# valeoai/rainbow-iqn-apex

Hardware: NVIDIA H100
Metric: learner grad-steps/sec (batch=512, N=N'=64) (higher is better)
Workload: dtype fp16 fwd / bf16 bwd tensor-core products, fp32 accumulate; fp32 elsewhere

## Files before the change

rainbow_iqn_apex_b200/csrc/conv.cu:

```cuda
#include "common.cuh"
#include "gemm.h"
#include "../../include/riqn_b200.h"

namespace riqn {

template <typename T>
__device__ __forceinline__ float load_px(const T* p);
template <>
__device__ __forceinline__ float load_px<uint8_t>(const uint8_t* p) { return (float)(*p) / 255.0f; }
template <>
__device__ __forceinline__ float load_px<float>(const float* p) { return *p; }

template <typename T>
__global__ void im2col_kernel(riqn_conv_geom g, const T* __restrict__ in, float* __restrict__ col) {
  const int K = g.Cin * g.KH * g.KW;
  const long total = (long)g.B * g.OH * g.OW * K;
  for (long idx = (long)blockIdx.x * blockDim.x + threadIdx.x; idx < total; idx += (long)gridDim.x * blockDim.x) {
    const int k = (int)(idx % K);
    const long m = idx / K;
    const int kw = k % g.KW, kh = (k / g.KW) % g.KH, c = k / (g.KW * g.KH);
    const int ow = (int)(m % g.OW), oh = (int)((m / g.OW) % g.OH), b = (int)(m / ((long)g.OW * g.OH));
    const int ih = oh * g.stride + kh - g.pad, iw = ow * g.stride + kw - g.pad;
    float v = 0.f;
    if (ih >= 0 && ih < g.H && iw >= 0 && iw < g.W) v = load_px<T>(&in[(long)b * g.in_bstride + ((long)c * g.H + ih) * g.W + iw]);
// ... 516 lines not shown
          d_[u][h] = on ? __ldg(dout + src) : 0.f;
        }
#pragma unroll
      for (int u = 0; u < 4; ++u) {
        const int c = c0 + 8 * u;
        if (c < Cout) {
          float acc = 0.f;
#pragma unroll
          for (int h = 0; h < 2; ++h) {
            const float v = o_[u][h] > 0.f ? d_[u][h] : 0.f;
            tile[lane + 32 * h][c] = __bfloat16_as_ushort(__float2bfloat16_rn(v));
            acc += v;
          }
          acc = warp_sum(acc);
          if (lane == 0) bsum[c] += acc;
        }
      }
    }
    __syncthreads();
    const int ppr = Cout >> 3;
    for (int idx = threadIdx.x; idx < 64 * ppr; idx += blockDim.x) {
      const int r = idx / ppr, pc = idx - r * ppr;
      if (m0 + r < Mg) {
        const uint32_t* w = reinterpret_cast<const uint32_t*>(&tile[r][pc * 8]);
        *reinterpret_cast<uint4*>(dYg + (m0 + r) * Cout + pc * 8) = make_uint4(w[0], w[1], w[2], w[3]);
      }
    }
    __syncthreads();
  }
  if (threadIdx.x < Cout) dbias_part[(long)blockIdx.x * Cout + threadIdx.x] = bsum[threadIdx.x];
}

__global__ void unpermute_add_kernel(int Cout, int K, const float* __restrict__ dwp, const int* __restrict__ perm,
                                     float* __restrict__ dw) {
  const int idx = blockIdx.x * blockDim.x + threadIdx.x;
  if (idx >= Cout * K) return;
  const int c = idx / K, kp = idx - c * K;
  dw[(long)c * K + perm[kp]] += dwp[idx];
}

static int strip_params(const riqn_conv_geom* g, int* t, int* G, int* kc) {
  if (g->KH != g->KW || g->stride < 1 || g->KH % g->stride) return 1;
  *t = g->KH / g->stride;
  *G = g->OH + *t - 1;
  const int Kc = g->stride * g->stride * g->Cin;
  if (g->OH != g->OW || Kc % 64 || g->OH != (g->H + 2 * g->pad - g->KH) / g->stride + 1) return 1;
  *kc = Kc / 64;
  return 0;
}

RIQN_API int riqn_s2d_u8(const riqn_conv_geom* g, const unsigned char* in, void* a_px, void* stream) {
  riqn::note_launches(1);
  int t, G, kc;
  const int chw = g->Cin * g->H * g->W;
  if (strip_params(g, &t, &G, &kc) || chw % 16 || g->in_bstride % 16 || (reinterpret_cast<uintptr_t>(in) & 15) ||
      chw > 96 * 1024)
    return (int)cudaErrorInvalidValue;
  static PerDeviceOnce attr_once;
  const int attr_dev = PerDeviceOnce::device();
  if (!attr_once.done[attr_dev]) {
    RIQN_CUDA(cudaFuncSetAttribute(s2d_u8_kernel, cudaFuncAttributeMaxDynamicSharedMemorySize, 96 * 1024));
    attr_once.done[attr_dev] = true;
  }
  s2d_u8_kernel<<<g->B, 256, chw, (cudaStream_t)stream>>>(*g, G, in, (bf16*)a_px);
  return (int)cudaGetLastError();
}

RIQN_API int riqn_conv_fwd_strip(const riqn_conv_geom* g, const void* a_hi, const void* a_lo, const void* w_hi,
                                 const void* w_lo, const float* bias, float* out, void* next_hi, void* next_lo,
                                 int next_stride, int next_grid, const void* w2_hi, const void* w2_lo, const float* bias2,
                                 int share_a, void* stream) {
  riqn::note_launches(1);
  int t, G, kc;
  if (strip_params(g, &t, &G, &kc) || g->Cout > 64 || (next_hi && (next_stride < 1 || next_grid < 1)))
    return (int)cudaErrorInvalidValue;
  TcExtra ex;
  if (w2_hi != nullptr) {
    const long rows = (long)g->B * G * G;
    if ((g->B & 1) || (rows / 2) % 128 || bias2 == nullptr || (w_lo != nullptr) != (w2_lo != nullptr)) return (int)cudaErrorInvalidValue;
    ex.grp_mt = (int)(rows / 2 / 128);
    ex.b2_hi = (const bf16*)w2_hi; ex.b2_lo = (const bf16*)w2_lo; ex.bias2 = bias2;
    if (share_a) { ex.a_wrap = 1; ex.a_rows = rows / 2; }
  }
  ex.strip_t = t; ex.strip_G = G; ex.strip_kc = kc;
  ex.cv_oh = g->OH; ex.cv_ow = g->OW;
  ex.nx_hi = (bf16*)next_hi; ex.nx_lo = (bf16*)next_lo; ex.nx_s = next_stride; ex.nx_G = next_grid;
  return gemm_bf16_tc(g->B * G * G, g->Cout, g->Cin * g->KH * g->KW, (const bf16*)a_hi, (const bf16*)a_lo, (const bf16*)w_hi,
                      (const bf16*)w_lo, out, g->Cout, TC_CONV, bias, nullptr, nullptr, 1, (cudaStream_t)stream, &ex);
}

__global__ void col2im_gather_kernel(riqn_conv_geom g, int G, const float* __restrict__ dcol, float* __restrict__ din) {
  const long i = (long)blockIdx.x * blockDim.x + threadIdx.x;
  const long n = (long)g.B * g.Cin * g.H * g.W;
  if (i >= n) return;
  const int c = (int)(i % g.Cin), iw = (int)((i / g.Cin) % g.W), ih = (int)((i / ((long)g.Cin * g.W)) % g.H);
  const long b = i / ((long)g.Cin * g.W * g.H);
  const int K = g.Cin * g.KH * g.KW;
  float acc = 0.f;
  for (int kh = 0; kh < g.KH; ++kh) {
    const int oy = ih - kh;
    if (oy < 0 || oy % g.stride) continue;
    const int oh = oy / g.stride;
    if (oh >= g.OH) continue;
    for (int kw = 0; kw < g.KW; ++kw) {
      const int ox = iw - kw;
      if (ox < 0 || ox % g.stride) continue;
      const int ow = ox / g.stride;
      if (ow >= g.OW) continue;
      acc += dcol[((b * G + oh) * G + ow) * K + (c * g.KH + kh) * g.KW + kw];
    }
  }
  din[((b * g.Cin + c) * g.H + ih) * g.W + iw] = acc;
}

RIQN_API int riqn_conv_bwd_strip(const riqn_conv_geom* g, const float* dout, const float* out, const void* a_hi,
                                 const void* w_hi, const int* perm, void* dYg, float* dwp_scratch, float* dw, float* dbias,
                                 float* din, float wgrad_scale, void* stream) {
  riqn::note_launches(din ? 6 : 4);
  cudaStream_t s = (cudaStream_t)stream;
  int t, G, kc;
  if (strip_params(g, &t, &G, &kc) || g->Cout > 64 || g->Cout % 8 || (din && g->pad != 0)) return (int)cudaErrorInvalidValue;
  const long Mg = (long)g->B * G * G;
  const int K = g->Cin * g->KH * g->KW;
  const long tiles = (Mg + 63) / 64;
  const int dy_grid = (int)(tiles < 4L * riqn_sms() ? tiles : 4L * riqn_sms());
  StreamScratch dbias_part;
  RIQN_CUDA(dbias_part.alloc((size_t)dy_grid * g->Cout, s));
  conv_dy_grid_kernel<<<dy_grid, 256, 0, s>>>(g->B, g->Cout, g->OH, g->OW, G, dout, out, (bf16*)dYg, dbias_part.p);
  RIQN_LAUNCH_CHECK();
  if (int rc_ = sum_slots_add(dy_grid, g->Cout, dbias_part.p, dbias, s)) return rc_;
  RIQN_CUDA(cudaMemsetAsync(dwp_scratch, 0, sizeof(float) * g->Cout * K, s));
  TcExtra ex;
  ex.mn_major = 3;
  ex.wg_t = t; ex.wg_G = G; ex.wg_kc = kc;
  ex.alpha = wgrad_scale;
  const int n_tiles = (K + 127) / 128;
  const int split = tc_pick_split(n_tiles, (Mg + 63) / 64);
  int rc = gemm_bf16_tc(g->Cout, K, (int)Mg, (const bf16*)dYg, nullptr, (const bf16*)a_hi, nullptr, dwp_scratch, K, TC_ATOMIC,
                        nullptr, nullptr, nullptr, split, s, &ex);
  if (rc) return rc;
  unpermute_add_kernel<<<(g->Cout * K + 255) / 256, 256, 0, s>>>(g->Cout, K, dwp_scratch, perm, dw);
  RIQN_LAUNCH_CHECK();
  if (din) {
    StreamScratch dcol_buf;
    RIQN_CUDA(dcol_buf.alloc((size_t)Mg * K, s));
    float* dcol = dcol_buf.p;
    TcExtra ci;
    ci.mn_major = 2;
    rc = gemm_bf16_tc((int)Mg, K, g->Cout, (const bf16*)dYg, nullptr, (const bf16*)w_hi, nullptr, dcol, K, TC_STORE, nullptr,
                      nullptr, nullptr, 1, s, &ci);
    if (rc) return rc;
    const long n_in = (long)g->B * g->Cin * g->H * g->W;
    col2im_gather_kernel<<<riqn_cdiv(n_in, 256), 256, 0, s>>>(*g, G, dcol, din);
    RIQN_LAUNCH_CHECK();
  }
  return 0;
}

RIQN_API int riqn_conv_bwd_tc(const riqn_conv_geom* g, const float* dout, const float* out, const void* colT_hi,
                              const void* wT_hi, void* dY_hi, void* dYT_hi, float* dcol, float* dw, float* dbias, float* din,
                              float wgrad_scale, void* stream) {
  riqn::note_launches(din ? 4 : 2);
  cudaStream_t s = (cudaStream_t)stream;
  const long M = (long)g->B * g->OH * g->OW;
  const int K = g->Cin * g->KH * g->KW;
  const int ohw = g->OH * g->OW;
  if (M % 8 || g->Cout % 8) return (int)cudaErrorInvalidValue;
  const long tiles = (M + 63) / 64;
  const int slots = g->Cout <= 64 ? (int)(tiles < 4L * riqn_sms() ? tiles : 4L * riqn_sms()) : (int)((M + 256 * 8 - 1) / (256 * 8));
  StreamScratch dbias_part;
  RIQN_CUDA(dbias_part.alloc((size_t)slots * g->Cout, s));
  if (g->Cout <= 64) {
    conv_dy_tile_kernel<<<slots, 256, 0, s>>>(g->B, g->Cout, ohw, dout, out, din ? (bf16*)dY_hi : nullptr, (bf16*)dYT_hi,
                                              dbias_part.p);
  } else {
    dim3 grid((unsigned)slots, g->Cout);
    conv_dy_bf16_kernel<<<grid, 256, 0, s>>>(g->B, g->Cout, ohw, dout, out, din ? (bf16*)dY_hi : nullptr, (bf16*)dYT_hi,
                                             dbias_part.p);
  }
  RIQN_LAUNCH_CHECK();
  if (int rc_ = sum_slots_add(slots, g->Cout, dbias_part.p, dbias, s)) return rc_;
  const int n_tiles = (K + 127) / 128;
  int split = (riqn_sms() + n_tiles - 1) / n_tiles;
  TcExtra ex;
  ex.alpha = wgrad_scale;
  int rc = gemm_bf16_tc(g->Cout, K, (int)M, (const bf16*)dYT_hi, nullptr, (const bf16*)colT_hi, nullptr, dw, K, TC_ATOMIC,
                        nullptr, nullptr, nullptr, split, s, &ex);
// ... 22 lines not shown
```

rainbow_iqn_apex_b200/csrc/gemm.h:

```cpp
#pragma once
#include <cuda_bf16.h>
#include <cuda_runtime.h>

#include "common.cuh"

namespace riqn {

enum Epi {
  EPI_STORE = 0,
  EPI_BIAS_RELU = 1,
  EPI_BIAS_RELU_NCHW = 2,
  EPI_EMBED = 3,
  EPI_ATOMIC = 4,
  EPI_NOISY_WGRAD = 5,
  EPI_BIAS = 6,
};

struct EpiArgs {
  const float* bias = nullptr;
  const float* feat = nullptr;
  int batch = 1;
  int ohw = 1;
  float* out2 = nullptr;
  const float* eps = nullptr;
  float alpha = 1.0f;
};

int gemm_f32(int M, int N, int K, const float* A, long sAm, long sAk, const float* B, long sBn, long sBk,
             float* C, long ldc, int epi, const EpiArgs& e, int split_k, cudaStream_t stream);

enum TcEpi { TC_STORE = 0, TC_BIAS_RELU = 1, TC_ATOMIC = 2, TC_NOISY_WGRAD = 3, TC_BIAS_RELU_NCHW = 4, TC_EMBED = 5,
             TC_COL2IM = 6, TC_CONV = 7 };

struct TcExtra {
  int ohw = 1;
  float alpha = 1.0f;
  const float* feat = nullptr;
  int batch = 1;
  __nv_bfloat16 *o_hi = nullptr, *o_lo = nullptr, *o_hiT = nullptr, *o_loT = nullptr;
  int ci_h = 0, ci_w = 0, ci_cin = 0, ci_kh = 0, ci_kw = 0, ci_stride = 0, ci_ow = 0, ci_G = 0, ci_oh = 0;
  int strip_t = 0, strip_G = 0, strip_kc = 0, cv_oh = 0, cv_ow = 0, nx_s = 0, nx_G = 0;
  __nv_bfloat16 *nx_hi = nullptr, *nx_lo = nullptr;
  int mn_major = 0, wg_t = 0, wg_G = 0, wg_kc = 0;
  int fmt = 0;
  int grp_mt = 0, a_wrap = 0;
  long a_rows = 0;
  const __nv_bfloat16 *b2_hi = nullptr, *b2_lo = nullptr;
  const float* bias2 = nullptr;
};

int gemm_bf16_tc(int M, int N, int K, const __nv_bfloat16* A_hi, const __nv_bfloat16* A_lo, const __nv_bfloat16* B_hi,
                 const __nv_bfloat16* B_lo, float* C, long ldc, int epi, const float* bias, float* out2, const float* eps,
                 int split_k, cudaStream_t s, const TcExtra* ex);
inline int tc_max_split(long tiles) {
  if (tiles < 1) tiles = 1;
  const long s = riqn_sms() / tiles;
  return s < 1 ? 1 : (int)s;
}
inline int tc_pick_split(int tiles, long kb) {
  const int s = tc_max_split(tiles);
  return kb < s ? (int)(kb < 1 ? 1 : kb) : s;
}

int split_bf16(long rows, int cols, const float* src, __nv_bfloat16* hi, __nv_bfloat16* lo, __nv_bfloat16* hiT,
               __nv_bfloat16* loT, cudaStream_t s, int fp16 = 0);
// ... 3 lines not shown
```

rainbow_iqn_apex_b200/csrc/gemm_tc.cu:

```cuda
#include <cuda.h>
#include <cudaTypedefs.h>
#include <algorithm>
#include <map>
#include <mutex>
#include <tuple>

#include "common.cuh"
#include "gemm.h"
#include "../../include/riqn_b200.h"

namespace riqn {

using bf16 = __nv_bfloat16;

constexpr int TBM = 128, TBK = 64, MMA_K = 16;
constexpr int kConsumerWGs = 2;
constexpr int kEpiWarps = 4 * kConsumerWGs;
constexpr int kTcThreads = 128 * (1 + kConsumerWGs);
constexpr uint32_t kSlabStride = 72, kSlabBytes = 64 * kSlabStride * 4;
constexpr uint32_t kSmemLimit = 232448;

template <int NSPLIT, int BN, int EPI>
struct TcCfg {
  static constexpr int kAOps = NSPLIT == 3 ? 2 : 1, kBOps = NSPLIT == 1 ? 1 : 2;
// ... 308 lines not shown
  uint64_t* bars = reinterpret_cast<uint64_t*>(smem + Cfg::kStages * Cfg::kStageBytes + Cfg::kEpiBytes);
  uint64_t* full = bars;
  uint64_t* empty = bars + Cfg::kStages;
  const uint32_t epi_base = (uint32_t)__cvta_generic_to_shared(smem + Cfg::kStages * Cfg::kStageBytes);
  const uint32_t epi_fb = epi_base + Cfg::kEpiBytes + 256;

  const int warp = threadIdx.x >> 5, lane = threadIdx.x & 31;
  const int total_units = p.m_tiles * p.n_tiles * p.k_splits;

  if (threadIdx.x == 0) {
    asm volatile("prefetch.tensormap [%0];" ::"l"(reinterpret_cast<uint64_t>(&mapA_hi)) : "memory");
    asm volatile("prefetch.tensormap [%0];" ::"l"(reinterpret_cast<uint64_t>(&mapB_hi)) : "memory");
    if (NSPLIT == 3) asm volatile("prefetch.tensormap [%0];" ::"l"(reinterpret_cast<uint64_t>(&mapA_lo)) : "memory");
    if (NSPLIT >= 2) asm volatile("prefetch.tensormap [%0];" ::"l"(reinterpret_cast<uint64_t>(&mapB_lo)) : "memory");
    for (int i = 0; i < Cfg::kStages; ++i) { mbar_init(&full[i], 1); mbar_init(&empty[i], kEpiWarps); }
    asm volatile("fence.mbarrier_init.release.cluster;" ::: "memory");
  }
  __syncthreads();

  if (warp < 4) {
    if constexpr (BN == 256) asm volatile("setmaxnreg.dec.sync.aligned.u32 40;" ::: "memory");
    if (warp == 0 && lane == 0) {
      int stage = 0;
      uint32_t phase = 0;
      for (int u = blockIdx.x; u < total_units; u += gridDim.x) {
        const int tiles = p.m_tiles * p.n_tiles;
        const int ks = u / tiles, t = u - ks * tiles;
        const int nt = t % p.n_tiles, mt = t / p.n_tiles;
        const int kb0 = ks * p.kb_per_split, kb1 = min(p.kb_total, kb0 + p.kb_per_split);
        for (int kb = kb0; kb < kb1; ++kb) {
          mbar_wait(&empty[stage], phase ^ 1);
          uint8_t* s = smem + stage * Cfg::kStageBytes;
          mbar_expect_tx(&full[stage], Cfg::kStageBytes);
          if (NSPLIT == 1 && p.mn_major) {
            const int kk = kb * TBK;
            if (p.mn_major & 1) {
#pragma unroll
              for (int i = 0; i < TBM / 64; ++i) tma_load_2d(s + i * 8192, &mapA_hi, mt * TBM + 64 * i, kk, &full[stage]);
            } else {
              tma_load_2d(s, &mapA_hi, kk, mt * TBM, &full[stage]);
            }
            if (p.mn_major & 2) {
#pragma unroll
              for (int i = 0; i < (TBN >= 64 ? TBN / 64 : 1); ++i) {
                int b_in = nt * TBN + 64 * i, b_row = kk;
                if (p.wg_t) {
                  const int slab = b_in >> 6, sft = slab / p.wg_kc, dy = sft / p.wg_t;
                  b_in = (slab - sft * p.wg_kc) << 6;
                  b_row += dy * p.wg_G + (sft - dy * p.wg_t);
                }
                tma_load_2d(s + Cfg::kOps * Cfg::kABytes + i * 8192, &mapB_hi, b_in, b_row, &full[stage]);
              }
            } else {
              tma_load_2d(s + Cfg::kOps * Cfg::kABytes, &mapB_hi, kk, nt * TBN, &full[stage]);
            }
            if (++stage == Cfg::kStages) { stage = 0; phase ^= 1; }
            continue;
          }
          int a_col = kb * TBK, a_row = mt * TBM;
          const CUtensorMap *mb_hi = &mapB_hi, *mb_lo = &mapB_lo;
          if (EPI == TC_CONV && p.grp_mt && mt >= p.grp_mt) {
            mb_hi = &p.mapO[0];
            mb_lo = &p.mapO[1];
            if (p.a_wrap) a_row = (mt - p.grp_mt) * TBM;
          }
          if (EPI == TC_CONV) {
// ... 12 lines not shown
    }
    return;
  }

  if constexpr (BN == 256) asm volatile("setmaxnreg.inc.sync.aligned.u32 232;" ::: "memory");
  const int g = (warp >> 2) - 1;
  const int wq = warp & 3;
  const int band = wq & 1, colhalf = wq >> 1;
  const int quarter = 2 * g + band;
  const int ew = warp - 4;
  const uint32_t slab = epi_base + g * kSlabBytes;
  const uint32_t st = slab + wq * (32 * kStRow * 4);
  const bool f16 = (p.fmt & 3) != 0;
  float conv_bias[32];
  if (EPI == TC_CONV) {
#pragma unroll
    for (int j = 0; j < 32; ++j) conv_bias[j] = (32 * colhalf + j < p.N && 32 * colhalf < TBN) ? p.bias[32 * colhalf + j] : 0.f;
  }
  bool conv_grp1 = false;
  int stage = 0;
  uint32_t phase = 0;
  for (int u = blockIdx.x; u < total_units; u += gridDim.x) {
    const int tiles = p.m_tiles * p.n_tiles;
    const int ks = u / tiles, t = u - ks * tiles;
    const int nt = t % p.n_tiles, mt = t / p.n_tiles;
    const int kb0 = ks * p.kb_per_split, kb1 = min(p.kb_total, kb0 + p.kb_per_split);
    if (EPI == TC_CONV && p.grp_mt && (mt >= p.grp_mt) != conv_grp1) {
      conv_grp1 = mt >= p.grp_mt;
      const float* bsrc = conv_grp1 ? p.bias2 : p.bias;
#pragma unroll
      for (int j = 0; j < 32; ++j) conv_bias[j] = (32 * colhalf + j < p.N && 32 * colhalf < TBN) ? bsrc[32 * colhalf + j] : 0.f;
    }
    float acc[TBN / 2];
    int prev = -1;
    for (int kb = kb0; kb < kb1; ++kb) {
      mbar_wait(&full[stage], phase);
      const uint32_t s0 = smem_u32(smem + stage * Cfg::kStageBytes);
      const uint32_t sa = s0 + g * 8192;
      const uint32_t sb = s0 + Cfg::kOps * Cfg::kABytes;
      wgmma_fence();
      if constexpr (BN == 256) {
        mma_kblock<TBN>(acc, sa, sb, kb == kb0, (MODE & 4) != 0, MODE & 3);
      } else if (NSPLIT == 1 && p.mn_major) {
#pragma unroll
        for (int k = 0; k < TBK / MMA_K; ++k) {
          const uint32_t koff_mn = k * (MMA_K / 8) * 1024;
          const uint32_t koff_k = k * MMA_K * 2;
          const uint64_t da = (p.mn_major & 1) ? gmma_desc_mn128(sa + koff_mn) : gmma_desc_k128(sa + koff_k);
          const uint64_t db = (p.mn_major & 2) ? gmma_desc_mn128(sb + koff_mn) : gmma_desc_k128(sb + koff_k);
          wgmma_tile<TBN>(acc, da, db, (kb > kb0 || k > 0) ? 1u : 0u, f16, p.mn_major);
        }
      } else {
#pragma unroll
        for (int k = 0; k < TBK / MMA_K; ++k) {
          const uint32_t koff = k * MMA_K * 2;
          const uint64_t a_hi = gmma_desc_k128(sa + koff), b_hi = gmma_desc_k128(sb + koff);
          wgmma_tile<TBN>(acc, a_hi, b_hi, (kb > kb0 || k > 0) ? 1u : 0u, f16, 0);
          if (NSPLIT >= 2) wgmma_tile<TBN>(acc, a_hi, gmma_desc_k128(sb + Cfg::kBBytes + koff), 1u, false, 0);
          if (NSPLIT == 3) wgmma_tile<TBN>(acc, gmma_desc_k128(sa + Cfg::kABytes + koff), b_hi, 1u, false, 0);
        }
      }
      wgmma_commit();
      wgmma_wait<1>();
      if (prev >= 0) {
        __syncwarp();
        if (lane == 0) mbar_arrive(&empty[prev]);
      }
      prev = stage;
      if (++stage == Cfg::kStages) { stage = 0; phase ^= 1; }
    }
    wgmma_wait<0>();
    __syncwarp();
    if (lane == 0) mbar_arrive(&empty[prev]);

#pragma unroll
    for (int h = 0; h < (TBN + 63) / 64; ++h) {
      if (BN == 256 && nt * TBN + 64 * h >= p.N) break;
      if (EPI == TC_EMBED && lane == 0) tma_store_wait_read();
      wg_bar(1 + g);
      {
        const uint32_t r0 = slab + ((16 * wq + (lane >> 2)) * kSlabStride + 2 * (lane & 3)) * 4;
#pragma unroll
        for (int j = 0; j < 8; ++j) {
          const int jj = 8 * h + j;
          if (jj * 8 < TBN) {
            asm volatile("st.shared.v2.f32 [%0], {%1, %2};" ::"r"(r0 + j * 32), "f"(acc[4 * jj]), "f"(acc[4 * jj + 1]) : "memory");
            asm volatile("st.shared.v2.f32 [%0], {%1, %2};" ::"r"(r0 + 8 * kSlabStride * 4 + j * 32), "f"(acc[4 * jj + 2]),
                         "f"(acc[4 * jj + 3]) : "memory");
          }
        }
      }
      wg_bar(1 + g);
      const int c = 64 * h + 32 * colhalf;
      uint32_t v[32];
      if (c < TBN) {
        const uint32_t rr = slab + ((32 * band + lane) * kSlabStride + 32 * colhalf) * 4;
#pragma unroll
        for (int j = 0; j < 8; ++j) {
          const uint4 x = lds128(rr + 16 * j);
          v[4 * j] = x.x; v[4 * j + 1] = x.y; v[4 * j + 2] = x.z; v[4 * j + 3] = x.w;
        }
      }
      wg_bar(1 + g);
      if (c >= TBN) continue;
      const int m = mt * TBM + quarter * 32 + lane;
      const int n0 = nt * TBN + c;
// ... 15 lines not shown
            for (int j = 0; j < 32; j += 4) {
              float4 o = make_float4(__uint_as_float(v[j]), __uint_as_float(v[j + 1]), __uint_as_float(v[j + 2]),
                                     __uint_as_float(v[j + 3]));
              if (EPI == TC_BIAS_RELU) {
                const float4 b = *reinterpret_cast<const float4*>(p.bias + n0 + j);
                o.x = fmaxf(o.x + b.x, 0.f); o.y = fmaxf(o.y + b.y, 0.f);
                o.z = fmaxf(o.z + b.z, 0.f); o.w = fmaxf(o.w + b.w, 0.f);
              }
              *reinterpret_cast<float4*>(crow + j) = o;
              if (EPI == TC_BIAS_RELU && p.o_hiT) {
                p.o_hiT[(long)(n0 + j) * p.M + m] = __float2bfloat16_rn(o.x);
                p.o_hiT[(long)(n0 + j + 1) * p.M + m] = __float2bfloat16_rn(o.y);
                p.o_hiT[(long)(n0 + j + 2) * p.M + m] = __float2bfloat16_rn(o.z);
                p.o_hiT[(long)(n0 + j + 3) * p.M + m] = __float2bfloat16_rn(o.w);
              }
            }
          } else {
#pragma unroll
            for (int j = 0; j < 32; ++j) {
              if (n0 + j < p.N) {
                float o = __uint_as_float(v[j]);
                if (EPI == TC_BIAS_RELU) o = fmaxf(o + p.bias[n0 + j], 0.f);
                crow[j] = o;
                if (EPI == TC_BIAS_RELU && p.o_hiT) p.o_hiT[(long)(n0 + j) * p.M + m] = __float2bfloat16_rn(o);
              }
            }
          }
        } else if (EPI == TC_BIAS_RELU_NCHW) {
          const int b = m / p.ohw, pp = m - b * p.ohw;
          float* cb = p.C + ((long)b * p.N + n0) * p.ohw + pp;
#pragma unroll
          for (int j = 0; j < 32; ++j)
            if (n0 + j < p.N) cb[(long)j * p.ohw] = fmaxf(__uint_as_float(v[j]) + p.bias[n0 + j], 0.f);
        } else if (EPI == TC_EMBED || EPI == TC_COL2IM || EPI == TC_CONV) {
        } else if (!(p.vec_acc && n0 + 32 <= p.N)) {
          float* crow = p.C + (long)m * p.ldc + n0;
#pragma unroll
          for (int j = 0; j < 32; ++j) {
            if (n0 + j < p.N) {
              const float o = __uint_as_float(v[j]) * (EPI == TC_ATOMIC ? p.alpha : 1.f);
              crow[j] += o;
              if (EPI == TC_NOISY_WGRAD) p.out2[(long)m * p.ldc + n0 + j] += o * p.eps[(long)m * p.ldc + n0 + j];
            }
          }
        }
      }
      if (EPI == TC_CONV && n0 < p.N) {
        const int gg = p.strip_G * p.strip_G;
        const int mm = m < p.M ? m : 0;
        const int b = mm / gg, rem = mm - b * gg;
        const int gy = rem / p.strip_G, gx = rem - gy * p.strip_G;
        const bool valid = m < p.M && gy < p.cv_oh && gx < p.cv_ow;
        float x[32];
#pragma unroll
        for (int j = 0; j < 32; ++j) x[j] = n0 + j < p.N ? fmaxf(__uint_as_float(v[j]) + conv_bias[j], 0.f) : 0.f;
        if (p.C != nullptr && valid) {
          const int plane = p.cv_oh * p.cv_ow;
          float* cb = p.C + ((long)b * p.N + n0) * plane + gy * p.cv_ow + gx;
#pragma unroll
          for (int j = 0; j < 32; ++j)
            if (n0 + j < p.N) cb[(long)j * plane] = x[j];
        }
        if (p.nx_hi != nullptr && n0 + 32 <= p.N) {
          long o = -1;
          if (valid) {
            const int sn = p.nx_s, by = gy / sn, bx = gx / sn;
            const long r = ((long)b * p.nx_G + by) * p.nx_G + bx;
// ... 12 lines not shown
          uint4 pc[8];
          long orow[8];
#pragma unroll
          for (int i = 0; i < 8; ++i) {
            pc[i] = staged_piece(st, 4 * i + sub, piece);
            orow[i] = __shfl_sync(0xffffffffu, o, 4 * i + sub);
          }
#pragma unroll
          for (int i = 0; i < 8; ++i)
            if (orow[i] >= 0 && dstb != nullptr) *reinterpret_cast<uint4*>(dstb + orow[i] + (piece & 3) * 8) = pc[i];
        }
      }
      if (EPI == TC_COL2IM && n0 < p.N) {
        const int khw = p.ci_kh * p.ci_kw;
        const int kcol = n0 + lane;
        int coff = -1;
        if (kcol < p.N) {
          const int c = kcol / khw, r = kcol - c * khw;
          const int kh = r / p.ci_kw, kw = r - kh * p.ci_kw;
          coff = (c * p.ci_h + kh) * p.ci_w + kw;
        }
        bool row_ok = m < p.M;
        const int mm = row_ok ? m : 0;
        const int b = mm / p.ohw, pp = mm - b * p.ohw;
        const int rw = p.ci_G ? p.ci_G : p.ci_ow;
        const int oh = pp / rw, ow = pp - oh * rw;
        if (p.ci_G) row_ok = row_ok && oh < p.ci_oh && ow < p.ci_ow;
        float* base = p.C + ((long)b * p.ci_cin * p.ci_h + oh * p.ci_stride) * p.ci_w + ow * p.ci_stride;
#pragma unroll
        for (int j = 0; j < 32; ++j) {
          const int off = __shfl_sync(0xffffffffu, coff, j);
          if (row_ok && off >= 0)
            asm volatile("red.global.add.f32 [%0], %1;" ::"l"(base + off), "f"(__uint_as_float(v[j])) : "memory");
        }
      }
      if ((EPI == TC_STORE || EPI == TC_EMBED || (EPI == TC_BIAS_RELU && (p.M & 1) == 0) ||
           ((EPI == TC_ATOMIC || EPI == TC_NOISY_WGRAD) && p.vec_acc)) && n0 + 32 <= p.N) {
        const int m_base = mt * TBM + quarter * 32;
        const int rows_valid = min(32, p.M - m_base);
        if (rows_valid > 0) {
          if (EPI == TC_STORE) {
            if (p.o_hi != nullptr) {
              uint32_t hw2[32];
#pragma unroll
              for (int j = 0; j < 16; ++j) {
                const __nv_bfloat162 h2 = __floats2bfloat162_rn(__uint_as_float(v[2 * j]), __uint_as_float(v[2 * j + 1]));
                hw2[j] = *reinterpret_cast<const uint32_t*>(&h2);
                hw2[16 + j] = 0u;
              }
              warp_store_rows_bf16(st, hw2, lane, p.o_hi + (long)m_base * p.N + n0, nullptr, p.N, rows_valid);
            } else {
              warp_store_rows_f32(st, v, lane, p.C + ks * p.part_stride + (long)m_base * p.ldc + n0, p.ldc, rows_valid);
            }
          } else if (EPI == TC_ATOMIC) {
            warp_accum_rows_f32<false>(st, v, lane, p.C + (long)m_base * p.ldc + n0, nullptr, nullptr, p.ldc, rows_valid,
                                       p.alpha);
          } else if (EPI == TC_NOISY_WGRAD) {
            const long o0 = (long)m_base * p.ldc + n0;
            warp_accum_rows_f32<true>(st, v, lane, p.C + o0, p.out2 + o0, p.eps + o0, p.ldc, rows_valid, 1.f);
          } else if (EPI == TC_BIAS_RELU) {
            const float* br = p.bias + n0;
            uint32_t hw[16];
#pragma unroll
            for (int j = 0; j < 32; j += 4) {
              const float4 bb = __ldg(reinterpret_cast<const float4*>(br + j));
              const float x0 = fmaxf(__uint_as_float(v[j]) + bb.x, 0.f), x1 = fmaxf(__uint_as_float(v[j + 1]) + bb.y, 0.f);
// ... 121 lines not shown
    attr_once.sms[attr_dev] = sms;
  }
  const int units = p.m_tiles * p.n_tiles * p.k_splits;
  const int grid = units < sms ? units : sms;
  gemm_tc_kernel<NSPLIT, EPI, BN, MODE><<<grid, kTcThreads, Cfg::kSmemBytes, s>>>(a_hi, a_lo, b_hi, b_lo, p);
  return (int)cudaGetLastError();
}

__global__ void split_k_reduce_kernel(int M, int N, int splits, long stride, long ldp, const float* __restrict__ part,
                                      float* __restrict__ C, long ldc, float alpha, float* __restrict__ out2,
                                      const float* __restrict__ eps) {
  const long i = (long)blockIdx.x * blockDim.x + threadIdx.x;
  if (i >= (long)M * N) return;
  const long m = i / N, n = i - m * N;
  float acc = 0.f;
  for (int k = 0; k < splits; ++k) acc += part[k * stride + m * ldp + n];
  C[m * ldc + n] += alpha * acc;
  if (out2 != nullptr) out2[m * ldc + n] += acc * eps[m * ldc + n];
}

int gemm_bf16_tc(int M, int N, int K, const bf16* A_hi, const bf16* A_lo, const bf16* B_hi, const bf16* B_lo, float* C,
                 long ldc, int epi, const float* bias, float* out2, const float* eps, int split_k, cudaStream_t s,
                 const TcExtra* ex) {
  if (M <= 0 || N <= 0 || K <= 0) return 0;
  if ((K % 8) && !(ex != nullptr && ex->mn_major == 3)) return (int)cudaErrorInvalidValue;
  const bool split3 = A_lo != nullptr && B_lo != nullptr;
  const bool split2 = A_lo == nullptr && B_lo != nullptr;
  const bool narrow_ok = epi == TC_BIAS_RELU_NCHW || epi == TC_CONV || ((epi == TC_ATOMIC || epi == TC_STORE) && !split3 && !split2);
  const bool strip = epi == TC_CONV;
  if (strip && (ex == nullptr || ex->strip_t < 1 || ex->strip_kc < 1 || ex->strip_G < 1 || N > 64 ||
                K != ex->strip_t * ex->strip_t * ex->strip_kc * TBK || (ex->nx_hi && (N % 32))))
    return (int)cudaErrorInvalidValue;
  const long a_k = strip ? (long)ex->strip_kc * TBK : K;
  const bool mn = ex != nullptr && ex->mn_major != 0;
  if (mn) {
    if (split3 || split2 || ((ex->mn_major & 1) && (M % 8)) || ((ex->mn_major & 2) && (N % 8)) ||
        (((ex->mn_major & 3) != 3) && (K % 8)))
      return (int)cudaErrorInvalidValue;
  }
  const long kb_all = (K + TBK - 1) / TBK;
  bool wide = false;
  if (!split3 && !split2 && N > 128 && kb_all >= 16 && (mn ? (ex->mn_major != 1 && ex->wg_t == 0) : !strip) &&
      (epi == TC_STORE || epi == TC_NOISY_WGRAD ||
       (epi == TC_BIAS_RELU && !mn && (ex == nullptr || ex->o_hiT == nullptr)))) {
    const long sms = riqn_sms();
    const long t128 = (long)((M + TBM - 1) / TBM) * ((N + 127) / 128), t256 = (long)((M + TBM - 1) / TBM) * ((N + 255) / 256);
    const bool unsplit = std::min(std::max(split_k, 1), std::min<int>(tc_max_split(t128), (int)kb_all)) == 1;
    wide = (epi != TC_NOISY_WGRAD || unsplit) && (t256 >= sms || 2 * ((t256 + sms - 1) / sms) <= (t128 + sms - 1) / sms);
  }
  const int bn = wide ? 256
                      : (ex != nullptr && ex->mn_major) ? ((narrow_ok && N <= 64) ? 64 : 128)
                                                        : (narrow_ok && N <= 32) ? 32 : (narrow_ok && N <= 64) ? 64 : 128;
  CUtensorMap ma_hi, ma_lo, mb_hi, mb_lo;
  int rc;
  if (mn) {
    const long b_cols = ex->wg_t ? (long)ex->wg_kc * TBK : N;
    rc = (ex->mn_major & 1) ? make_map(&ma_hi, A_hi, K, M, 64) : make_map(&ma_hi, A_hi, M, K, TBM);
    if (rc) return rc;
    rc = (ex->mn_major & 2) ? make_map(&mb_hi, B_hi, K, b_cols, 64) : make_map(&mb_hi, B_hi, N, K, bn);
    if (rc) return rc;
  } else {
    rc = make_map(&ma_hi, A_hi, (ex && ex->a_rows) ? ex->a_rows : M, a_k, TBM);
    if (rc) return rc;
    rc = make_map(&mb_hi, B_hi, N, K, bn);
    if (rc) return rc;
  }
  ma_lo = ma_hi;
  mb_lo = mb_hi;
  if (split3) {
    rc = make_map(&ma_lo, A_lo, (ex && ex->a_rows) ? ex->a_rows : M, a_k, TBM);
    if (rc) return rc;
  }
  if (split3 || split2) {
    rc = make_map(&mb_lo, B_lo, N, K, bn);
    if (rc) return rc;
  }
  TcArgs p;
  p.M = M; p.N = N; p.K = K;
  p.m_tiles = (M + TBM - 1) / TBM;
  p.n_tiles = (N + bn - 1) / bn;
  p.kb_total = (K + TBK - 1) / TBK;
  if (split_k < 1) split_k = 1;
  if (split_k > tc_max_split(p.m_tiles * p.n_tiles)) split_k = tc_max_split(p.m_tiles * p.n_tiles);
  if (split_k > p.kb_total) split_k = p.kb_total;
  p.kb_per_split = (p.kb_total + split_k - 1) / split_k;
  p.k_splits = (p.kb_total + p.kb_per_split - 1) / p.kb_per_split;
  if (p.k_splits > 1 && epi != TC_ATOMIC && epi != TC_NOISY_WGRAD) return (int)cudaErrorInvalidValue;
  p.C = C; p.ldc = ldc; p.bias = bias; p.out2 = out2; p.eps = eps; p.part_stride = 0;
  p.alpha = ex ? ex->alpha : 1.f;
  p.vec_acc = (ldc % 4 == 0) && (reinterpret_cast<uintptr_t>(C) & 15) == 0 && (reinterpret_cast<uintptr_t>(out2) & 15) == 0 &&
              (reinterpret_cast<uintptr_t>(eps) & 15) == 0;
  p.ohw = ex ? ex->ohw : 1; p.feat = ex ? ex->feat : nullptr; p.batch = ex ? ex->batch : 1;
  p.ci_h = ex ? ex->ci_h : 0; p.ci_w = ex ? ex->ci_w : 0; p.ci_cin = ex ? ex->ci_cin : 0; p.ci_kh = ex ? ex->ci_kh : 0;
  p.ci_kw = ex ? ex->ci_kw : 0; p.ci_stride = ex ? ex->ci_stride : 0; p.ci_ow = ex ? ex->ci_ow : 0;
  p.ci_G = ex ? ex->ci_G : 0; p.ci_oh = ex ? ex->ci_oh : 0;
  p.strip_t = ex ? ex->strip_t : 0; p.strip_G = ex ? ex->strip_G : 0; p.strip_kc = ex ? ex->strip_kc : 0;
  p.cv_oh = ex ? ex->cv_oh : 0; p.cv_ow = ex ? ex->cv_ow : 0; p.nx_s = ex ? ex->nx_s : 0; p.nx_G = ex ? ex->nx_G : 0;
  p.nx_hi = ex ? ex->nx_hi : nullptr; p.nx_lo = ex ? ex->nx_lo : nullptr;
  p.mn_major = mn ? ex->mn_major : 0; p.wg_t = ex ? ex->wg_t : 0; p.wg_G = ex ? ex->wg_G : 0; p.wg_kc = ex ? ex->wg_kc : 0;
  if (epi == TC_COL2IM && (ex == nullptr || p.ci_kh * p.ci_kw * p.ci_cin != N || split3 || split2)) return (int)cudaErrorInvalidValue;
  p.o_hi = ex ? ex->o_hi : nullptr; p.o_lo = ex ? ex->o_lo : nullptr;
  p.o_hiT = ex ? ex->o_hiT : nullptr; p.o_loT = ex ? ex->o_loT : nullptr;
  p.fmt = ex ? ex->fmt : 0;
  p.grp_mt = ex ? ex->grp_mt : 0; p.a_wrap = ex ? ex->a_wrap : 0; p.bias2 = ex ? ex->bias2 : nullptr;
  if (p.grp_mt) {
    if (epi != TC_CONV || !ex->b2_hi || !ex->bias2 || p.m_tiles != 2 * p.grp_mt || (split3 || split2) != (ex->b2_lo != nullptr))
      return (int)cudaErrorInvalidValue;
    if ((rc = make_map(&p.mapO[0], ex->b2_hi, N, K, bn))) return rc;
    p.mapO[1] = p.mapO[0];
    if (ex->b2_lo && (rc = make_map(&p.mapO[1], ex->b2_lo, N, K, bn))) return rc;
  }
  if ((p.fmt & 3) && (split3 || split2)) return (int)cudaErrorInvalidValue;
  if ((p.fmt & 3) == 1 || (p.fmt & 3) == 2) return (int)cudaErrorInvalidValue;
  if ((p.fmt & 4) && epi != TC_EMBED) return (int)cudaErrorInvalidValue;
// ... 7 lines not shown
#define RIQN_TC_NARROW(NS, EP)                                                                  \
    if (bn == 32) return launch_tc<NS, EP, 32>(ma_hi, ma_lo, mb_hi, mb_lo, p, s);                  \
    if (bn == 64) return launch_tc<NS, EP, 64>(ma_hi, ma_lo, mb_hi, mb_lo, p, s)
    if (split3) {
      switch (epi) {
        case TC_STORE: RIQN_TC_GO(3, TC_STORE);
        case TC_BIAS_RELU: RIQN_TC_GO(3, TC_BIAS_RELU);
        case TC_ATOMIC: RIQN_TC_GO(3, TC_ATOMIC);
        case TC_NOISY_WGRAD: RIQN_TC_GO(3, TC_NOISY_WGRAD);
        case TC_BIAS_RELU_NCHW: RIQN_TC_NARROW(3, TC_BIAS_RELU_NCHW); RIQN_TC_GO(3, TC_BIAS_RELU_NCHW);
        case TC_CONV: RIQN_TC_NARROW(3, TC_CONV); break;
        case TC_EMBED: RIQN_TC_GO(3, TC_EMBED);
      }
    } else if (split2) {
      switch (epi) {
        case TC_BIAS_RELU_NCHW: RIQN_TC_NARROW(2, TC_BIAS_RELU_NCHW); RIQN_TC_GO(2, TC_BIAS_RELU_NCHW);
        case TC_CONV: RIQN_TC_NARROW(2, TC_CONV); break;
        case TC_STORE: RIQN_TC_GO(2, TC_STORE);
        default: return (int)cudaErrorInvalidValue;
      }
    } else if (bn == 256) {
      const int mode = p.mn_major | ((p.fmt & 3) ? 4 : 0);
#define RIQN_TC_WIDE(EP, MD) if (epi == EP && mode == MD) return launch_tc<1, EP, 256, MD>(ma_hi, ma_lo, mb_hi, mb_lo, p, s)
      RIQN_TC_WIDE(TC_BIAS_RELU, 0); RIQN_TC_WIDE(TC_BIAS_RELU, 4);
      RIQN_TC_WIDE(TC_STORE, 0); RIQN_TC_WIDE(TC_STORE, 2); RIQN_TC_WIDE(TC_STORE, 3);
      RIQN_TC_WIDE(TC_STORE, 4); RIQN_TC_WIDE(TC_STORE, 6); RIQN_TC_WIDE(TC_STORE, 7);
      RIQN_TC_WIDE(TC_NOISY_WGRAD, 0); RIQN_TC_WIDE(TC_NOISY_WGRAD, 2); RIQN_TC_WIDE(TC_NOISY_WGRAD, 3);
      RIQN_TC_WIDE(TC_NOISY_WGRAD, 4); RIQN_TC_WIDE(TC_NOISY_WGRAD, 6); RIQN_TC_WIDE(TC_NOISY_WGRAD, 7);
#undef RIQN_TC_WIDE
    } else {
      switch (epi) {
        case TC_STORE: RIQN_TC_NARROW(1, TC_STORE); RIQN_TC_GO(1, TC_STORE);
        case TC_COL2IM: RIQN_TC_GO(1, TC_COL2IM);
        case TC_BIAS_RELU: RIQN_TC_GO(1, TC_BIAS_RELU);
        case TC_ATOMIC: RIQN_TC_NARROW(1, TC_ATOMIC); RIQN_TC_GO(1, TC_ATOMIC);
        case TC_NOISY_WGRAD: RIQN_TC_GO(1, TC_NOISY_WGRAD);
        case TC_BIAS_RELU_NCHW: RIQN_TC_NARROW(1, TC_BIAS_RELU_NCHW); RIQN_TC_GO(1, TC_BIAS_RELU_NCHW);
        case TC_CONV: RIQN_TC_NARROW(1, TC_CONV); break;
        case TC_EMBED: RIQN_TC_GO(1, TC_EMBED);
      }
    }
#undef RIQN_TC_NARROW
#undef RIQN_TC_GO
    return (int)cudaErrorInvalidValue;
  };
  if (p.k_splits == 1) return go(epi);
  const long ldp = (N + 3) & ~3L;
  StreamScratch part;
  RIQN_CUDA(part.alloc((size_t)p.k_splits * M * ldp, s));
  const float alpha = epi == TC_ATOMIC ? p.alpha : 1.f;
  p.C = part.p;
  p.ldc = ldp;
  p.part_stride = (long)M * ldp;
  p.o_hi = nullptr;
  if ((rc = go(TC_STORE))) return rc;
  const long n = (long)M * N;
  split_k_reduce_kernel<<<riqn_cdiv(n, 256), 256, 0, s>>>(M, N, p.k_splits, p.part_stride, ldp, part.p, C, ldc, alpha,
                                                          epi == TC_NOISY_WGRAD ? out2 : nullptr, eps);
  return (int)cudaGetLastError();
}

__global__ void split_bf16_kernel(long rows, int cols, const float* __restrict__ src, bf16* __restrict__ hi,
                                  bf16* __restrict__ lo, bf16* __restrict__ hiT, bf16* __restrict__ loT, int fp16) {
  __shared__ float tile[32][33];
  const long r0 = (long)blockIdx.y * 32;
  const int c0 = blockIdx.x * 32;
// ... 131 lines not shown
```

Baseline: 219.6.

## Fuse conv input-grad col2im into tensor-core GEMM with shifted-row TMA loads

Replaces the conv input-gradient path, a full dcol GEMM followed by a col2im gather kernel, with a new TC_CONV_DGRAD GEMM epilogue. Each k-block loads A rows shifted by the strip offset and a matching slice of the permuted weight. The per-offset products are summed in registers and written straight to the input gradient in space-to-depth layout. The unpermute kernel also gathers a permuted bf16 weight copy, which removes the large dcol scratch buffer and one launch. In exchange it waits for every wgmma after each k-block, which serialises the MMA pipeline, and it adds stricter geometry constraints.

```diff
diff --git a/rainbow_iqn_apex_b200/csrc/conv.cu b/rainbow_iqn_apex_b200/csrc/conv.cu
--- a/rainbow_iqn_apex_b200/csrc/conv.cu
+++ b/rainbow_iqn_apex_b200/csrc/conv.cu
@@ -572,11 +572,13 @@
 }
 
 __global__ void unpermute_add_kernel(int Cout, int K, const float* __restrict__ dwp, const int* __restrict__ perm,
-                                     float* __restrict__ dw) {
+                                     float* __restrict__ dw, const bf16* __restrict__ w_hi, bf16* __restrict__ w_s) {
   const int idx = blockIdx.x * blockDim.x + threadIdx.x;
   if (idx >= Cout * K) return;
   const int c = idx / K, kp = idx - c * K;
-  dw[(long)c * K + perm[kp]] += dwp[idx];
+  const long o = (long)c * K + perm[kp];
+  dw[o] += dwp[idx];
+  if (w_s) w_s[idx] = w_hi[o];
 }
 
 static int strip_params(const riqn_conv_geom* g, int* t, int* G, int* kc) {
@@ -629,37 +631,15 @@
                       (const bf16*)w_lo, out, g->Cout, TC_CONV, bias, nullptr, nullptr, 1, (cudaStream_t)stream, &ex);
 }
 
-__global__ void col2im_gather_kernel(riqn_conv_geom g, int G, const float* __restrict__ dcol, float* __restrict__ din) {
-  const long i = (long)blockIdx.x * blockDim.x + threadIdx.x;
-  const long n = (long)g.B * g.Cin * g.H * g.W;
-  if (i >= n) return;
-  const int c = (int)(i % g.Cin), iw = (int)((i / g.Cin) % g.W), ih = (int)((i / ((long)g.Cin * g.W)) % g.H);
-  const long b = i / ((long)g.Cin * g.W * g.H);
-  const int K = g.Cin * g.KH * g.KW;
-  float acc = 0.f;
-  for (int kh = 0; kh < g.KH; ++kh) {
-    const int oy = ih - kh;
-    if (oy < 0 || oy % g.stride) continue;
-    const int oh = oy / g.stride;
-    if (oh >= g.OH) continue;
-    for (int kw = 0; kw < g.KW; ++kw) {
-      const int ox = iw - kw;
-      if (ox < 0 || ox % g.stride) continue;
-      const int ow = ox / g.stride;
-      if (ow >= g.OW) continue;
-      acc += dcol[((b * G + oh) * G + ow) * K + (c * g.KH + kh) * g.KW + kw];
-    }
-  }
-  din[((b * g.Cin + c) * g.H + ih) * g.W + iw] = acc;
-}
-
 RIQN_API int riqn_conv_bwd_strip(const riqn_conv_geom* g, const float* dout, const float* out, const void* a_hi,
                                  const void* w_hi, const int* perm, void* dYg, float* dwp_scratch, float* dw, float* dbias,
                                  float* din, float wgrad_scale, void* stream) {
-  riqn::note_launches(din ? 6 : 4);
+  riqn::note_launches(din ? 5 : 4);
   cudaStream_t s = (cudaStream_t)stream;
   int t, G, kc;
-  if (strip_params(g, &t, &G, &kc) || g->Cout > 64 || g->Cout % 8 || (din && g->pad != 0)) return (int)cudaErrorInvalidValue;
+  if (strip_params(g, &t, &G, &kc) || g->Cout > 64 || g->Cout % 8 ||
+      (din && (g->pad != 0 || g->H != g->W || G * g->stride != g->H)))
+    return (int)cudaErrorInvalidValue;
   const long Mg = (long)g->B * G * G;
   const int K = g->Cin * g->KH * g->KW;
   const long tiles = (Mg + 63) / 64;
@@ -679,20 +659,18 @@
   int rc = gemm_bf16_tc(g->Cout, K, (int)Mg, (const bf16*)dYg, nullptr, (const bf16*)a_hi, nullptr, dwp_scratch, K, TC_ATOMIC,
                         nullptr, nullptr, nullptr, split, s, &ex);
   if (rc) return rc;
-  unpermute_add_kernel<<<(g->Cout * K + 255) / 256, 256, 0, s>>>(g->Cout, K, dwp_scratch, perm, dw);
+  StreamScratch w_s;
+  if (din) RIQN_CUDA(w_s.alloc(((size_t)g->Cout * K + 1) / 2, s));
+  unpermute_add_kernel<<<(g->Cout * K + 255) / 256, 256, 0, s>>>(g->Cout, K, dwp_scratch, perm, dw, (const bf16*)w_hi,
+                                                                 (bf16*)w_s.p);
   RIQN_LAUNCH_CHECK();
   if (din) {
-    StreamScratch dcol_buf;
-    RIQN_CUDA(dcol_buf.alloc((size_t)Mg * K, s));
-    float* dcol = dcol_buf.p;
-    TcExtra ci;
-    ci.mn_major = 2;
-    rc = gemm_bf16_tc((int)Mg, K, g->Cout, (const bf16*)dYg, nullptr, (const bf16*)w_hi, nullptr, dcol, K, TC_STORE, nullptr,
-                      nullptr, nullptr, 1, s, &ci);
+    TcExtra dg;
+    dg.strip_t = t; dg.strip_G = G;
+    dg.ci_cin = g->Cin; dg.ci_h = g->H; dg.ci_w = g->W; dg.ci_stride = g->stride;
+    rc = gemm_bf16_tc((int)Mg, kc * 64, g->Cout, (const bf16*)dYg, nullptr, (const bf16*)w_s.p, nullptr, din, 0,
+                      TC_CONV_DGRAD, nullptr, nullptr, nullptr, 1, s, &dg);
     if (rc) return rc;
-    const long n_in = (long)g->B * g->Cin * g->H * g->W;
-    col2im_gather_kernel<<<riqn_cdiv(n_in, 256), 256, 0, s>>>(*g, G, dcol, din);
-    RIQN_LAUNCH_CHECK();
   }
   return 0;
 }
diff --git a/rainbow_iqn_apex_b200/csrc/gemm.h b/rainbow_iqn_apex_b200/csrc/gemm.h
--- a/rainbow_iqn_apex_b200/csrc/gemm.h
+++ b/rainbow_iqn_apex_b200/csrc/gemm.h
@@ -30,7 +30,7 @@
              float* C, long ldc, int epi, const EpiArgs& e, int split_k, cudaStream_t stream);
 
 enum TcEpi { TC_STORE = 0, TC_BIAS_RELU = 1, TC_ATOMIC = 2, TC_NOISY_WGRAD = 3, TC_BIAS_RELU_NCHW = 4, TC_EMBED = 5,
-             TC_COL2IM = 6, TC_CONV = 7 };
+             TC_COL2IM = 6, TC_CONV = 7, TC_CONV_DGRAD = 8 };
 
 struct TcExtra {
   int ohw = 1;
diff --git a/rainbow_iqn_apex_b200/csrc/gemm_tc.cu b/rainbow_iqn_apex_b200/csrc/gemm_tc.cu
--- a/rainbow_iqn_apex_b200/csrc/gemm_tc.cu
+++ b/rainbow_iqn_apex_b200/csrc/gemm_tc.cu
@@ -364,6 +364,15 @@
           mbar_wait(&empty[stage], phase ^ 1);
           uint8_t* s = smem + stage * Cfg::kStageBytes;
           mbar_expect_tx(&full[stage], Cfg::kStageBytes);
+          if constexpr (EPI == TC_CONV_DGRAD) {
+            const int dy = kb / p.strip_t, dx = kb - dy * p.strip_t;
+            tma_load_2d(s, &mapA_hi, 0, mt * TBM - (dy * p.strip_G + dx), &full[stage]);
+#pragma unroll
+            for (int i = 0; i < TBN / 64; ++i)
+              tma_load_2d(s + Cfg::kABytes + i * 8192, &mapB_hi, kb * p.N + nt * TBN + 64 * i, 0, &full[stage]);
+            if (++stage == Cfg::kStages) { stage = 0; phase ^= 1; }
+            continue;
+          }
           if (NSPLIT == 1 && p.mn_major) {
             const int kk = kb * TBK;
             if (p.mn_major & 1) {
@@ -442,6 +451,11 @@
       for (int j = 0; j < 32; ++j) conv_bias[j] = (32 * colhalf + j < p.N && 32 * colhalf < TBN) ? bsrc[32 * colhalf + j] : 0.f;
     }
     float acc[TBN / 2];
+    float dg_sum[TBN / 2];
+    if constexpr (EPI == TC_CONV_DGRAD) {
+#pragma unroll
+      for (int i = 0; i < TBN / 2; ++i) dg_sum[i] = 0.f;
+    }
     int prev = -1;
     for (int kb = kb0; kb < kb1; ++kb) {
       mbar_wait(&full[stage], phase);
@@ -449,7 +463,9 @@
       const uint32_t sa = s0 + g * 8192;
       const uint32_t sb = s0 + Cfg::kOps * Cfg::kABytes;
       wgmma_fence();
-      if constexpr (BN == 256) {
+      if constexpr (EPI == TC_CONV_DGRAD) {
+        mma_kblock<TBN>(acc, sa, sb, true, false, 2);
+      } else if constexpr (BN == 256) {
         mma_kblock<TBN>(acc, sa, sb, kb == kb0, (MODE & 4) != 0, MODE & 3);
       } else if (NSPLIT == 1 && p.mn_major) {
 #pragma unroll
@@ -478,10 +494,19 @@
       }
       prev = stage;
       if (++stage == Cfg::kStages) { stage = 0; phase ^= 1; }
+      if constexpr (EPI == TC_CONV_DGRAD) {
+        wgmma_wait<0>();
+#pragma unroll
+        for (int i = 0; i < TBN / 2; ++i) dg_sum[i] += acc[i];
+      }
     }
     wgmma_wait<0>();
     __syncwarp();
     if (lane == 0) mbar_arrive(&empty[prev]);
+    if constexpr (EPI == TC_CONV_DGRAD) {
+#pragma unroll
+      for (int i = 0; i < TBN / 2; ++i) acc[i] = dg_sum[i];
+    }
 
 #pragma unroll
     for (int h = 0; h < (TBN + 63) / 64; ++h) {
@@ -563,7 +588,7 @@
 #pragma unroll
           for (int j = 0; j < 32; ++j)
             if (n0 + j < p.N) cb[(long)j * p.ohw] = fmaxf(__uint_as_float(v[j]) + p.bias[n0 + j], 0.f);
-        } else if (EPI == TC_EMBED || EPI == TC_COL2IM || EPI == TC_CONV) {
+        } else if (EPI == TC_EMBED || EPI == TC_COL2IM || EPI == TC_CONV || EPI == TC_CONV_DGRAD) {
         } else if (!(p.vec_acc && n0 + 32 <= p.N)) {
           float* crow = p.C + (long)m * p.ldc + n0;
 #pragma unroll
@@ -642,6 +667,23 @@
           const int off = __shfl_sync(0xffffffffu, coff, j);
           if (row_ok && off >= 0)
             asm volatile("red.global.add.f32 [%0], %1;" ::"l"(base + off), "f"(__uint_as_float(v[j])) : "memory");
+        }
+      }
+      if (EPI == TC_CONV_DGRAD && n0 < p.N) {
+        const int kcol = n0 + lane, s = p.ci_stride;
+        int coff = -1;
+        if (kcol < p.N) {
+          const int blk = kcol / p.ci_cin, c = kcol - blk * p.ci_cin, iy = blk / s, ix = blk - iy * s;
+          coff = (c * p.ci_h + iy) * p.ci_w + ix;
+        }
+        const bool row_ok = m < p.M;
+        const int gg = p.strip_G * p.strip_G, mm = row_ok ? m : 0;
+        const int b = mm / gg, rem = mm - b * gg, gy = rem / p.strip_G, gx = rem - gy * p.strip_G;
+        float* base = p.C + ((long)b * p.ci_cin * p.ci_h + gy * s) * p.ci_w + gx * s;
+#pragma unroll
+        for (int j = 0; j < 32; ++j) {
+          const int off = __shfl_sync(0xffffffffu, coff, j);
+          if (row_ok && off >= 0) base[off] = __uint_as_float(v[j]);
         }
       }
       if ((EPI == TC_STORE || EPI == TC_EMBED || (EPI == TC_BIAS_RELU && (p.M & 1) == 0) ||
@@ -829,6 +871,11 @@
                 K != ex->strip_t * ex->strip_t * ex->strip_kc * TBK || (ex->nx_hi && (N % 32))))
     return (int)cudaErrorInvalidValue;
   const long a_k = strip ? (long)ex->strip_kc * TBK : K;
+  const bool dgrad = epi == TC_CONV_DGRAD;
+  if (dgrad && (ex == nullptr || split3 || split2 || ex->mn_major || ex->strip_t < 1 || ex->strip_G < 1 || K > TBK ||
+                N % 64 || split_k > 1 || ex->ci_cin < 1 || ex->ci_stride < 1 || N != ex->ci_stride * ex->ci_stride * ex->ci_cin ||
+                ex->ci_h != ex->strip_G * ex->ci_stride || ex->ci_w != ex->ci_h))
+    return (int)cudaErrorInvalidValue;
   const bool mn = ex != nullptr && ex->mn_major != 0;
   if (mn) {
     if (split3 || split2 || ((ex->mn_major & 1) && (M % 8)) || ((ex->mn_major & 2) && (N % 8)) ||
@@ -846,11 +893,16 @@
     wide = (epi != TC_NOISY_WGRAD || unsplit) && (t256 >= sms || 2 * ((t256 + sms - 1) / sms) <= (t128 + sms - 1) / sms);
   }
   const int bn = wide ? 256
-                      : (ex != nullptr && ex->mn_major) ? ((narrow_ok && N <= 64) ? 64 : 128)
-                                                        : (narrow_ok && N <= 32) ? 32 : (narrow_ok && N <= 64) ? 64 : 128;
+                      : (dgrad || (ex != nullptr && ex->mn_major)) ? ((dgrad || narrow_ok) && N <= 64 ? 64 : 128)
+                                                                   : (narrow_ok && N <= 32) ? 32 : (narrow_ok && N <= 64) ? 64 : 128;
   CUtensorMap ma_hi, ma_lo, mb_hi, mb_lo;
   int rc;
-  if (mn) {
+  if (dgrad) {
+    rc = make_map(&ma_hi, A_hi, M, K, TBM);
+    if (rc) return rc;
+    rc = make_map(&mb_hi, B_hi, K, (long)ex->strip_t * ex->strip_t * N, 64);
+    if (rc) return rc;
+  } else if (mn) {
     const long b_cols = ex->wg_t ? (long)ex->wg_kc * TBK : N;
     rc = (ex->mn_major & 1) ? make_map(&ma_hi, A_hi, K, M, 64) : make_map(&ma_hi, A_hi, M, K, TBM);
     if (rc) return rc;
@@ -876,7 +928,7 @@
   p.M = M; p.N = N; p.K = K;
   p.m_tiles = (M + TBM - 1) / TBM;
   p.n_tiles = (N + bn - 1) / bn;
-  p.kb_total = (K + TBK - 1) / TBK;
+  p.kb_total = dgrad ? ex->strip_t * ex->strip_t : (K + TBK - 1) / TBK;
   if (split_k < 1) split_k = 1;
   if (split_k > tc_max_split(p.m_tiles * p.n_tiles)) split_k = tc_max_split(p.m_tiles * p.n_tiles);
   if (split_k > p.kb_total) split_k = p.kb_total;
@@ -950,6 +1002,9 @@
       switch (epi) {
         case TC_STORE: RIQN_TC_NARROW(1, TC_STORE); RIQN_TC_GO(1, TC_STORE);
         case TC_COL2IM: RIQN_TC_GO(1, TC_COL2IM);
+        case TC_CONV_DGRAD:
+          if (bn == 64) return launch_tc<1, TC_CONV_DGRAD, 64>(ma_hi, ma_lo, mb_hi, mb_lo, p, s);
+          RIQN_TC_GO(1, TC_CONV_DGRAD);
         case TC_BIAS_RELU: RIQN_TC_GO(1, TC_BIAS_RELU);
         case TC_ATOMIC: RIQN_TC_NARROW(1, TC_ATOMIC); RIQN_TC_GO(1, TC_ATOMIC);
         case TC_NOISY_WGRAD: RIQN_TC_GO(1, TC_NOISY_WGRAD);
```

New measurement: 239.6, median of 6. 1.09x the previous value.
